# Ogeon/pyrite

Measured on AMD Instinct MI355X. Metric: Msamples/sec, higher is better.
Workload: dtype f32; 1 GPU; C3: c3_mesh_in_box, 1920x1080, 1024 spp; bounces=8, light_samples=4, spectrum_samples=10, spectrum_bins=64, tile_size=32, triangles=819212, spheres=0, parallelism=one launch on one GPU, film_weight_check=ok

## Files before the change

pyrite_amd/csrc/api.cpp:

```cpp
#include <hip/hip_runtime.h>

#include <algorithm>
#include <chrono>
#include <cmath>
#include <cstdlib>
#include <cstring>
#include <memory>
#include <new>
#include <string>
#include <vector>

#include "api_internal.h"
#include "bvh.h"
#include "bvh_device.h"
#include "device_scene.h"
#include "program_regs.h"
#include "scene_internal.h"

using namespace pyr;

namespace pyr {

thread_local std::string g_error;
int fail(int code, const std::string& message) {
// ... 710 lines not shown
            } else if (pr.fast != FAST_NONE) {
                bool seen = false;
                for (size_t j = 0; j < i && !seen; ++j) {
                    const DevProgram& q = programs[j];
                    seen = q.kind == PYR_PROGRAM_INSTRUCTIONS && q.fast == pr.fast && q.fast_spectrum == pr.fast_spectrum && std::memcmp(&q.fast_scale, &pr.fast_scale, sizeof(float)) == 0;
                }
                fast_programs += seen ? 0u : 1u;
            }
        }
    }
    if (needs_interpreter) {
        bool ok = programs.size() <= 128;
        auto colour = [&](uint32_t id) {
            if (id >= programs.size()) return;
            const DevProgram& pr = programs[id];
            if (pr.kind != PYR_PROGRAM_INSTRUCTIONS) return;
            if (pr.tape_form == TAPE_FORM_NONE) ok = false;
            if (pr.tape_form == TAPE_FORM_HIT_RGB) v.rgb_records = 1u;
            if (pr.tape_form == TAPE_FORM_HIT_RGB || pr.tape_form == TAPE_FORM_PRODUCT) v.micro_records = 1u;
            if (pr.tape_form == TAPE_FORM_PRODUCT) v.product_records = 1u;
        };
        for (uint32_t i = 0; i < d->num_components; ++i) colour(d->components[i].color_program);
        for (uint32_t i = 0; i < d->num_lamps; ++i)
            if (d->lamps[i].kind != PYR_LAMP_SHAPE) colour(d->lamps[i].color_program);
        colour(d->sky_program);
        if (tape_rows_needed(fast_programs, v.rgb_records != 0) > kTapeMaxValueRows) ok = false;
        const char* off = std::getenv("PYRITE_HIT_TAPE");
        if (off && off[0] == '0') ok = false;
        if (wide_vm) ok = false;
        v.hit_tape = ok ? 1u : 0u;
        if (!ok) v.rgb_records = v.micro_records = v.product_records = 0u;
    }
    v.tape_value_rows = tape_rows_needed(fast_programs, v.rgb_records != 0) <= kTapeMaxValueRows ? tape_rows_needed(fast_programs, v.rgb_records != 0) : kTapeValueRows;
    v.shadow_margin = d->num_spheres != 0 ? 1.01f : 1.001f;
    v.hero_only_records = 0;
    for (uint32_t i = 0; i < d->num_materials; ++i)
        for (uint32_t k = 0; k < d->materials[i].num_emissive; ++k) {
            const int probability = d->components[d->materials[i].first_emissive + k].probability_program;
            if (probability >= 0 && programs[(size_t)probability].reads_wavelength) v.hero_only_records = 1u;
        }
    v.sphere_tex_scale = (const float*)s->sphere_tex_scale.ptr;
    v.plane_frames = (const float*)s->plane_frames.ptr;
    v.textures = (const DevTexture*)s->textures.ptr;
    v.texture_data = (const float*)s->texture_data.ptr;

    if ((rc = pack_geometry(d, s, builder)) != PYR_OK) return rc;
    s->live.keep(d);
    PyrBuildInfo& build_info = s->build_info;
    build_info.total_ms = (float)ms_between(t_start, std::chrono::steady_clock::now());
    build_info.pack_upload_ms = build_info.total_ms - build_info.bounds_ms - build_info.tree_ms - build_info.finish_ms - build_info.collapse_ms;
    return PYR_OK;
}

uint64_t film_buffer_grains(const PyrFilmDesc* film, const PyrRenderParams* p, const TilePlan& plan) {
    if (p->film_layout == PYR_FILM_TILE_BLOCKS) return (uint64_t)plan.tile_count * (p->tile_size + 2ull) * (p->tile_size + 2ull) * film->bins;
    const uint32_t rows = p->film_row_count ? p->film_row_count : film->height;
    return (uint64_t)rows * film->width * film->bins;
}


int reserve_tape(PyrScene* scene, RenderLaunch& L, hipStream_t stream) {
    const size_t bytes = (size_t)L.tape_lanes * L.tape_max_ops * sizeof(unsigned long long);
    if (bytes > scene->tape.bytes) {
        HIP_TRY(hipStreamSynchronize(stream));
        scene->tape.release();
        int rc = scene->tape.alloc(bytes);
// ... 566 lines not shown
```

pyrite_amd/csrc/device_scene.h:

```cpp
#pragma once
#include <cstddef>
#include <cstdint>

#include "../../include/pyrite_gpu.h"

namespace pyr {

struct DevPrim {
    float a[4], b[4], c[4];
};

struct DevPrimPair {
    float q[5][4];
};

struct DevTriShade {
    float n1[4], n2[4], n3[4];
};

struct DevTriTex {
    float uv12[4], uv3[4], f1[4], f2[4], f3[4];
};

struct DevTexture {
// ... 61 lines not shown
    float rgb_min, rgb_max;
    uint32_t sky_program;
    uint32_t stack_depth;
    uint32_t needs_interpreter;
    uint32_t num_nodes, num_prims;
    uint32_t num_spectra, num_spectrum_floats;
    uint32_t num_programs;
    uint32_t num_materials, num_components;
    uint32_t lds_table_floats;
    const float* tri_tex;
    const float* sphere_tex_scale;
    const float* plane_frames;
    const DevTexture* textures;
    const float* texture_data;
    uint32_t uses_textures;
    uint32_t hero_only_records;
    uint32_t hit_tape;
    uint32_t rgb_records;
    uint32_t product_records;
    uint32_t micro_records;
    float shadow_margin;
    uint32_t tape_value_rows;
};

constexpr uint32_t kTapeValueRows = 8, kTapeOneRow = kTapeValueRows - 1, kTapeMaxValueRows = 16;
constexpr uint32_t tape_row(uint32_t slot) { return slot + (slot >= kTapeOneRow ? 1u : 0u); }
constexpr uint32_t tape_rgb_row(uint32_t n_spectral) { return n_spectral + 3u <= kTapeOneRow ? n_spectral : (n_spectral >= kTapeOneRow ? n_spectral + 1u : kTapeValueRows); }
constexpr uint32_t tape_rows_needed(uint32_t n_spectral, bool rgb) {
    return (rgb ? tape_rgb_row(n_spectral) + 3u : (n_spectral == 0u ? 0u : tape_row(n_spectral - 1u) + 1u)) > kTapeValueRows
               ? (rgb ? tape_rgb_row(n_spectral) + 3u : tape_row(n_spectral - 1u) + 1u)
               : kTapeValueRows;
}

constexpr uint32_t kMaxStackDepth = 64;

struct RenderLaunch {
    PyrCamera camera;
    PyrFilmDesc film;
    uint32_t bounces, light_samples, spectrum_samples, tile_size, pixel_samples;
    uint32_t tiles_x, tiles_y;
    uint32_t tile_begin, tile_stride, tile_count;
    uint32_t chunks_per_tile;
    uint32_t chunk_begin, chunk_end;
    uint32_t film_layout;
    uint32_t film_row_begin, film_row_count;
    uint64_t seed;
    float grains_per_wavelength;
    PyrGrain* film_out;
    unsigned long long* counters;
    uint32_t scheduler;
    uint32_t sm_phase_lanes, sm_trav_steps;
    uint32_t sm_expose_lanes;
    uint32_t stack_lds;
    unsigned long long* tape;
    uint32_t tape_lanes, tape_max_ops;
    uint32_t* tape_overflow;
    uint32_t tape_programs_lds;
    uint32_t sample_begin;
    uint32_t* start_queue;
    uint32_t start_queue_stride;
};

#ifndef PYR_SAMPLE_QUEUE
#define PYR_SAMPLE_QUEUE 1
#endif
constexpr uint32_t kStartQueueEntries = 128, kStartQueueFixedWords = 11;
// ... 207 lines not shown
```

pyrite_amd/csrc/kernels.hip:

```cpp
#ifndef PYRITE_KERNELS_HIP
#define PYRITE_KERNELS_HIP
#include <hip/hip_runtime.h>

#include <algorithm>
#include <cstdint>
#include <cstdlib>
#include <string>
#include <type_traits>

#include "device_scene.h"
#include "exact_math.h"

#ifdef PYR_WIDE_VM
#define PYR_VM_NUMBERS PYR_WIDE_NUMBER_REGISTERS
#define PYR_VM_VECTORS PYR_WIDE_VECTOR_REGISTERS
#define PYR_VM_RGBS PYR_WIDE_RGB_REGISTERS
#else
#define PYR_VM_NUMBERS PYR_MAX_NUMBER_REGISTERS
#define PYR_VM_VECTORS PYR_MAX_VECTOR_REGISTERS
#define PYR_VM_RGBS PYR_MAX_RGB_REGISTERS
#endif
static_assert((PYR_VM_NUMBERS & (PYR_VM_NUMBERS - 1)) == 0 && (PYR_VM_VECTORS & (PYR_VM_VECTORS - 1)) == 0 && (PYR_VM_RGBS & (PYR_VM_RGBS - 1)) == 0,
              "the interpreter masks register indices: its files are powers of two");

// ... 1930 lines not shown
        const uint32_t first = code >> 3, count = code & 7u;
        const ScenePtr<true> pr{view.pairs + 5 * (size_t)first};
        const bool blocks = leaf_pair_test<COUNT>(pr[0], pr[1], pr[2], pr[3], pr[4], count, t, cnt);
        const bool more = count > 2u;
        done = blocks | (!more & (t.sp == 0));
        t.node = more ? -1 - (int)(((first + 1u) << 3) | (count - 2u)) : top;
        t.sp = more ? t.sp : below;
    }
    return done;
}

#ifndef PYR_PRIO_E
#define PYR_PRIO_E 0
#endif
#ifndef PYR_PRIO_S
#define PYR_PRIO_S 1
#endif
#ifndef PYR_PRIO_N
#define PYR_PRIO_N 2
#endif
#ifndef PYR_PRIO_T
#define PYR_PRIO_T 3
#endif
#define PYR_PRIO_ANY (PYR_PRIO_E != PYR_PRIO_S || PYR_PRIO_S != PYR_PRIO_N || PYR_PRIO_N != PYR_PRIO_T)
#if PYR_PRIO_ANY
#define PHASE_PRIO(x) __builtin_amdgcn_s_setprio(x)
#else
#define PHASE_PRIO(x)
#endif

constexpr uint32_t kTapeEagerSlots = 8;
constexpr uint32_t TAPE_MUL = 0u, TAPE_ADD = 1u, TAPE_SCALE = 2u, TAPE_HERO_ONLY = 1u << 29, TAPE_PROGRAM_MASK = (1u << 28) - 1u;
constexpr uint32_t TAPE_EAGER_ADD = 1u << 31, TAPE_EAGER_SLOT_SHIFT = 8, TAPE_EAGER_SLOT_MASK = 0xFu << TAPE_EAGER_SLOT_SHIFT;
constexpr uint32_t kTapeOneSlot = kTapeEagerSlots - 1;
static_assert(kTapeEagerSlots == kTapeValueRows && kTapeOneSlot == kTapeOneRow, "device_scene.h tape_row() and friends");
constexpr uint32_t TAPE_RGB_SHIFT = 12, TAPE_RGB_FIRST = 1u << TAPE_RGB_SHIFT, TAPE_RGB_NEXT = 2u << TAPE_RGB_SHIFT, TAPE_RGB_APPLY = 3u << TAPE_RGB_SHIFT,
                   TAPE_RGB_TIMES = 4u << TAPE_RGB_SHIFT;
static_assert(BLOCK == 1u << TAPE_EAGER_SLOT_SHIFT, "an eager record's slot field is an index into rows of BLOCK floats");

DEV size_t tape_index(uint32_t op, uint32_t lanes, uint32_t column) { return (size_t)op * lanes + column; }
template <bool COUNT, bool INTERP, bool TAPE = false, bool PRODUCT = false>
struct Walker {
    uint32_t stage = ST_NEW;
    uint32_t n_ops = 0;
    uint32_t tape_column = 0;
    const uint32_t* tape_prepared = nullptr;
    DEV void tape_push(const RenderLaunch& L, uint32_t kind, uint32_t program, float s, bool hero_only = false) {
        if (n_ops < L.tape_max_ops) {
            uint32_t word = (kind << 30) | (hero_only ? TAPE_HERO_ONLY : 0u) | (program & TAPE_PROGRAM_MASK);
            if (tape_prepared != nullptr) {
                uint32_t slot = kTapeOneSlot;
                if (kind != TAPE_SCALE) {
                    const uint32_t* e = tape_prepared + 8 * program;
                    if (e[0] == 0u)
                        s = __uint_as_float(e[1]) * s;
                    else
                        slot = e[7];
                }
                word = (kind == TAPE_ADD ? TAPE_EAGER_ADD : 0u) | (hero_only ? TAPE_HERO_ONLY : 0u) | (slot << TAPE_EAGER_SLOT_SHIFT);
            }
            L.tape[tape_index(n_ops, L.tape_lanes, tape_column)] = (unsigned long long)word | ((unsigned long long)__float_as_uint(s) << 32);
        } else {
            *L.tape_overflow = 1u;
        }
        n_ops++;
    }
    DEV void tape_push_raw(const RenderLaunch& L, uint32_t word, float s) {
        if (n_ops < L.tape_max_ops)
            L.tape[tape_index(n_ops, L.tape_lanes, tape_column)] = (unsigned long long)word | ((unsigned long long)__float_as_uint(s) << 32);
        else
            *L.tape_overflow = 1u;
        n_ops++;
    }
    uint32_t rgb_slot = 0;
    static constexpr bool QUEUE = PYR_SAMPLE_QUEUE != 0 && TAPE && !INTERP;
    uint32_t chunk = 0;
    uint32_t q_state = 0;
#ifdef PYR_PHASE_PROFILE
    unsigned long long prof_start[4] = {0, 0, 0, 0};
#endif
    Path p{};
    Trav t{};
    f3 b_position = mk(0, 0, 0), b_normal = mk(0, 0, 0), b_out = mk(0, 0, 0);
    bool b_flip = false;
// ... 372 lines not shown
    for (uint32_t k = 0; k < p.num_instrs; ++k) {
        const PyrInstr& ins = S.instrs[p.first_instr + k];
        float r = 0.0f;
        switch (ins.op) {
        case PYR_OP_NUMBER: r = __uint_as_float(ins.x.bits); break;
        case PYR_OP_SPECTRUM: r = spectrum_get(S, ins.a, value(ins.x)); break;
        case PYR_OP_BLACKBODY: {
            const float wl = value(ins.x), temp = value(ins.y);
            r = blackbody(wl, temp);
            break;
        }
        case PYR_OP_MIX: {
            const float amount = fmaxf(fminf(value(ins.x), 1.0f), 0.0f);
            const float l = num[ins.a & (PYR_MAX_NUMBER_REGISTERS - 1)], rr = num[ins.b & (PYR_MAX_NUMBER_REGISTERS - 1)];
            r = l * (1.0f - amount) + rr * amount;
            break;
        }
        case PYR_OP_BINARY: {
            const float l = num[ins.a & (PYR_MAX_NUMBER_REGISTERS - 1)], rr = num[ins.b & (PYR_MAX_NUMBER_REGISTERS - 1)];
            r = ins.operator_ == PYR_BIN_ADD ? l + rr : (ins.operator_ == PYR_BIN_SUB ? l - rr : (ins.operator_ == PYR_BIN_MUL ? l * rr : l / rr));
            break;
        }
        default: {
            const float v = value(ins.x), mn = value(ins.y), mx = value(ins.z);
            r = fmaxf(fminf(v, mx), mn);
            break;
        }
        }
        num[ins.output & (PYR_MAX_NUMBER_REGISTERS - 1)] = r;
    }
    return num[p.output_reg & (PYR_MAX_NUMBER_REGISTERS - 1)];
}

template <bool COUNT, bool RGB = false, bool TIMES = false>
DEV void replay_tapes(const DevScene& S, const RenderLaunch& L, bool exposing, uint32_t n_ops, uint32_t tape_column, const Path& p, const float* wl_rows,
                      uint32_t wl_column, uint32_t* wave_list, const uint32_t* prepared_lds, float* spectral_values, uint32_t n_spectral, bool eager, Counters& cnt) {
    const uint32_t lane = threadIdx.x & 63u;
    const unsigned long long mask = ballot64(exposing);
    const uint32_t n = (uint32_t)__popcll(mask);
    if (n == 0) return;
    uint32_t max_ops = exposing ? (n_ops < L.tape_max_ops ? n_ops : L.tape_max_ops) : 0u;
    const uint32_t my_ops = max_ops;
    for (int off = 32; off > 0; off >>= 1) max_ops = max(max_ops, (uint32_t)__shfl_xor((int)max_ops, off));
    const bool keeps = exposing && p.use_additional, lost = exposing && !p.use_additional;
    const bool longest = 3u * my_ops > 2u * max_ops, shortest = 3u * my_ops <= max_ops;
    const unsigned long long below = (1ull << lane) - 1ull;
    const unsigned long long k0 = ballot64(keeps && longest), k1 = ballot64(keeps && !longest && !shortest), k2 = ballot64(keeps && shortest);
    const unsigned long long l0 = ballot64(lost && longest), l1 = ballot64(lost && !longest && !shortest), l2 = ballot64(lost && shortest);
    const uint32_t n_full = (uint32_t)__builtin_popcountll(k0 | k1 | k2);
    if (exposing) {
        const unsigned long long mine = keeps ? (longest ? k0 : (shortest ? k2 : k1)) : (longest ? l0 : (shortest ? l2 : l1));
        uint32_t before = keeps ? 0u : n_full;
        before += (uint32_t)__builtin_popcountll(keeps ? ((longest ? 0ull : k0) | (shortest ? k1 : 0ull)) : ((longest ? 0ull : l0) | (shortest ? l1 : 0ull)));
        wave_list[before + (uint32_t)__builtin_popcountll(mine & below)] = lane;
    }
    __builtin_amdgcn_wave_barrier();
    const uint32_t SS = L.spectrum_samples, full_items = n_full * SS, items = full_items + (n - n_full);
    const unsigned long long past_the_end =
        eager ? ((unsigned long long)(kTapeOneSlot << TAPE_EAGER_SLOT_SHIFT) | ((unsigned long long)__float_as_uint(1.0f) << 32)) : 0ull;
#ifndef PYR_REPLAY_ROWS
#define PYR_REPLAY_ROWS 8
#endif
    constexpr uint32_t ROWS = PYR_REPLAY_ROWS;
    for (uint32_t base = 0; base < items; base += 64) {
        const uint32_t i = base + lane;
        const bool active = i < items;
        const bool full = i < full_items;
        const uint32_t rank = !active ? 0u : (full ? i / SS : n_full + (i - full_items)), k = !active ? 0u : (full ? i - rank * SS : SS - 1u);
        const uint32_t src = wave_list[rank];
        const uint32_t ops = (uint32_t)__shfl((int)n_ops, (int)src);
        uint32_t pass_ops = active ? (ops < L.tape_max_ops ? ops : L.tape_max_ops) : 0u;
        for (int off = 32; off > 0; off >>= 1) pass_ops = max(pass_ops, (uint32_t)__shfl_xor((int)pass_ops, off));
        const uint32_t pixel = (uint32_t)__shfl((int)p.pixel, (int)src);
        const float hero_wl = __shfl(p.wl, (int)src);
        const bool hero = k == SS - 1;
        const bool run = active;
        const uint32_t src_column = (uint32_t)__shfl((int)wl_column, (int)src);
        const float wl = hero ? hero_wl : wl_rows[k * BLOCK + src_column];
        float refl = 1.0f, bright = 0.0f, value = 0.0f;
        uint32_t value_of = 0xFFFFFFFFu;
        [[maybe_unused]] float rgb_sum = 0.0f;
        if (eager) {
            const uint32_t* slot_program = prepared_lds + 8 * L.tape_programs_lds;
            uint32_t grid_min = 0, grid_max = 0, grid_count = 0;
            uint32_t i0 = 0, i1 = 0;
            float mix = 0.0f;
            bool below = false, above = false;
            for (uint32_t slot = 0; slot < n_spectral; ++slot) {
                const uint32_t* e = prepared_lds + 8 * slot_program[slot];
                const uint32_t mode = e[0], format = e[2], count = e[6];
                const float c = __uint_as_float(e[1]);
                const float* data = S.spectrum_data + e[5];
                float v;
                if (RGB && mode == 0xFFu) {
                    v = lambda_eval(S, S.programs[slot_program[slot]], wl);
                } else if (format == PYR_SPECTRUM_ARRAY && count != 0u) {
                    if (e[3] != grid_min || e[4] != grid_max || count != grid_count) {
                        grid_min = e[3], grid_max = e[4], grid_count = count;
                        const float lo = __uint_as_float(grid_min), hi = __uint_as_float(grid_max);
                        below = wl <= lo, above = wl >= hi;
                        const float normalized = (wl - lo) / (hi - lo);
                        const float float_index = normalized * ((float)count - 1.0f);
                        const float min_float_index = truncf(float_index);
                        i0 = (below | above) ? 0u : (uint32_t)min_float_index;
                        i1 = (below | above) ? 0u : i0 + 1u;
                        mix = float_index - min_float_index;
                    }
                    const float inside = data[i0] * (1.0f - mix) + data[i1] * mix;
                    v = below ? data[0] : (above ? data[count - 1] : inside);
                } else {
                    PyrSpectrum sp;
                    sp.format = format, sp.min = __uint_as_float(e[3]), sp.max = __uint_as_float(e[4]), sp.offset = e[5], sp.count = count;
                    v = spectrum_eval(sp, data, wl);
                }
                spectral_values[tape_row(slot) * BLOCK] = (mode == FAST_SPECTRUM || mode == 0xFFu) ? v : v * c;
            }
            if (RGB && S.rgb_records != 0) {
                float resp[3] = {0.0f, 0.0f, 0.0f};
                const uint32_t count = S.rgb_count;
                if (count > 0) {
                    const float* d = S.rgb_basis;
                    if (wl <= S.rgb_min) {
                        for (int j = 0; j < 3; ++j) resp[j] = d[j];
                    } else if (wl >= S.rgb_max) {
                        for (int j = 0; j < 3; ++j) resp[j] = d[3 * (count - 1) + j];
                    } else {
                        const float normalized = (wl - S.rgb_min) / (S.rgb_max - S.rgb_min);
                        const float fi = normalized * ((float)count - 1.0f);
                        const float fmin_ = truncf(fi);
                        const uint32_t b0 = (uint32_t)fmin_;
                        const float bmix = fi - fmin_;
                        for (int j = 0; j < 3; ++j) resp[j] = d[3 * b0 + j] * (1.0f - bmix) + d[3 * (b0 + 1) + j] * bmix;
                    }
                }
                for (uint32_t j = 0; j < 3; ++j) spectral_values[(tape_rgb_row(n_spectral) + j) * BLOCK] = resp[j];
            }
        }
        for (uint32_t r0 = 0; r0 < pass_ops; r0 += ROWS) {
            unsigned long long rows[ROWS];
#pragma unroll
            for (uint32_t j = 0; j < ROWS; ++j) rows[j] = r0 + j < my_ops ? L.tape[tape_index(r0 + j, L.tape_lanes, tape_column)] : past_the_end;
            uint32_t words[ROWS];
            float factors[ROWS];
#pragma unroll
            for (uint32_t j = 0; j < ROWS; ++j) {
                words[j] = (uint32_t)__shfl((int)(uint32_t)rows[j], (int)src);
                factors[j] = __uint_as_float((uint32_t)__shfl((int)(uint32_t)(rows[j] >> 32), (int)src));
            }
// ... 56 lines not shown
                if ((word & TAPE_HERO_ONLY) && !hero) continue;
                const uint32_t program = word & TAPE_PROGRAM_MASK;
                if (program != value_of) {
                    Prepared q_prog;
                    if (program < L.tape_programs_lds) {
                        const uint32_t* e = prepared_lds + 8 * program;
                        q_prog.mode = e[0];
                        q_prog.c = __uint_as_float(e[1]);
                        q_prog.sp.format = e[2];
                        q_prog.sp.min = __uint_as_float(e[3]);
                        q_prog.sp.max = __uint_as_float(e[4]);
                        q_prog.sp.offset = e[5];
                        q_prog.sp.count = e[6];
                        q_prog.data = S.spectrum_data + e[5];
                        q_prog.id = program;
                    } else {
                        q_prog = prepare_program<false>(S, program);
                    }
                    VmInput in{wl, mk(0, 0, 0), mk(0, 0, 0)};
                    value = eval_prepared<false>(S, q_prog, in);
                    value_of = program;
                }
                if (kind == TAPE_MUL)
                    refl *= value * s;
                else
                    bright += value * s * refl;
            }
        }
        if (run) expose_grain<COUNT>(L, pixel, wl, bright, cnt);
    }
    __builtin_amdgcn_wave_barrier();
}

DEV uint32_t prepare_tape_tables(const DevScene& S0, const DevScene& S, const RenderLaunch& L, uint32_t* prepared_lds, bool& eager) {
    auto reads_spectrum = [&](uint32_t i) {
        return S0.programs[i].kind != PYR_PROGRAM_CONSTANT && (S0.programs[i].fast != FAST_NONE || (S0.hit_tape != 0 && S0.programs[i].tape_form == TAPE_FORM_LAMBDA));
    };
    auto alike = [&](uint32_t i, uint32_t j) {
        const DevProgram &a = S0.programs[i], &b = S0.programs[j];
        return a.fast != FAST_NONE && a.fast == b.fast && __float_as_uint(a.fast_scale) == __float_as_uint(b.fast_scale) && a.fast_spectrum == b.fast_spectrum;
    };
    auto first_alike = [&](uint32_t i) {
        for (uint32_t j = 0; j < i; ++j)
            if (reads_spectrum(j) && alike(i, j)) return j;
        return i;
    };
    auto slot_of = [&](uint32_t representative) {
        uint32_t slot = 0;
        for (uint32_t j = 0; j < representative; ++j) slot += (reads_spectrum(j) && first_alike(j) == j) ? 1u : 0u;
        return slot;
    };
    uint32_t n_spectral = 0;
    for (uint32_t i = 0; i < L.tape_programs_lds; ++i) n_spectral += (reads_spectrum(i) && first_alike(i) == i) ? 1u : 0u;
    for (uint32_t i = threadIdx.x; i < L.tape_programs_lds; i += BLOCK) {
        const Prepared q = prepare_program<false>(S, i);
        const bool spectral = reads_spectrum(i);
        const uint32_t representative = spectral ? first_alike(i) : i;
        const uint32_t slot = spectral ? slot_of(representative) : 0u;
        uint32_t* e = prepared_lds + 8 * i;
        e[0] = q.mode, e[1] = __float_as_uint(q.c), e[2] = q.sp.format, e[3] = __float_as_uint(q.sp.min), e[4] = __float_as_uint(q.sp.max);
        e[5] = q.sp.offset, e[6] = q.sp.count, e[7] = tape_row(slot);
        if (spectral && representative == i && slot < kTapeMaxValueRows - 1u) prepared_lds[8 * L.tape_programs_lds + slot] = i;
    }
    __syncthreads();
    eager = L.tape_programs_lds != 0 && tape_rows_needed(n_spectral, S0.rgb_records != 0) <= S0.tape_value_rows && (n_spectral != 0 || S0.hit_tape != 0);
    return eager ? n_spectral : 0u;
}

#ifndef PYR_SM_WAVES_INTERP
#define PYR_SM_WAVES_INTERP 3
#endif
constexpr int sm_waves(bool interp) { return interp ? PYR_SM_WAVES_INTERP : PYR_SM_WAVES; }
template <bool COUNT, bool INTERP, bool LDS_SCENE, bool LDS_TABLES, bool HIT_TAPE = false, bool PRODUCT = false>
__global__ __launch_bounds__(BLOCK, sm_waves(INTERP)) void render_kernel_sm(DevScene S0, RenderLaunch L) {
    extern __shared__ float lds[];
    static_assert(INTERP || !HIT_TAPE, "HIT_TAPE is a form of the interpreter build");
    static_assert(HIT_TAPE || !PRODUCT, "PRODUCT is a form of the hit tape (device_scene.h TapeForm)");
    constexpr bool TAPE = !INTERP || HIT_TAPE;
    const uint32_t SS = L.spectrum_samples;
    Spectral spec{lds + threadIdx.x, SS};
    const uint32_t spectral_rows = TAPE ? SS + 1 + S0.tape_value_rows : 3 * SS;
    TravStack stack;
    int deep_levels[LDS_SCENE ? 1 : kMaxStackDepth];
    stack.deep = deep_levels;
    stack.lds = (lds_int*)(reinterpret_cast<int*>(lds + spectral_rows * BLOCK) + threadIdx.x);
    constexpr bool QUEUE = Walker<COUNT, INTERP, TAPE, PRODUCT>::QUEUE;
    stack.lds_entries = QUEUE ? (int)own_scalar(L.stack_lds) : (int)L.stack_lds;
    Counters cnt{};
    const uint32_t lds_base_floats = (spectral_rows + L.stack_lds) * BLOCK;
    const SceneView view = stage_scene<LDS_SCENE>(S0, lds, lds_base_floats, true);
    const DevScene S = stage_tables<LDS_TABLES ? 1 : 0>(S0, lds, lds_base_floats + (LDS_SCENE ? (S0.num_nodes * 16 + S0.num_prims * 12) : 0));

    const uint32_t lane = threadIdx.x & 63u;
    const uint32_t waves_per_block = BLOCK / 64;
    const uint32_t total_waves = gridDim.x * waves_per_block;
    const int phase_lanes = QUEUE ? (int)own_scalar(L.sm_phase_lanes) : (int)L.sm_phase_lanes, trav_steps = QUEUE ? (int)own_scalar(L.sm_trav_steps) : (int)L.sm_trav_steps;
    const int expose_lanes = TAPE ? (QUEUE ? (int)own_scalar(L.sm_expose_lanes) : (int)L.sm_expose_lanes) : phase_lanes;
    Walker<COUNT, INTERP, TAPE, PRODUCT> w;
    w.chunk = L.chunk_begin + blockIdx.x * waves_per_block + (threadIdx.x >> 6);
    w.tape_prepared = nullptr;
    uint32_t* wave_list = reinterpret_cast<uint32_t*>(lds + SS * BLOCK) + (threadIdx.x & ~63u);
    uint32_t* prepared_lds = reinterpret_cast<uint32_t*>(lds + lds_base_floats + (LDS_SCENE ? (S0.num_nodes * 16 + S0.num_prims * 12) : 0) + (LDS_TABLES ? S0.lds_table_floats : 0));
    uint32_t n_spectral = 0;
    bool eager = false;
    float* spectral_values = lds + (SS + 1) * BLOCK + threadIdx.x;
    if constexpr (TAPE) {
        spectral_values[kTapeOneSlot * BLOCK] = 1.0f;
        n_spectral = prepare_tape_tables(S0, S, L, prepared_lds, eager);
        if (eager) w.tape_prepared = prepared_lds;
        w.rgb_slot = tape_rgb_row(n_spectral);
        w.tape_column = blockIdx.x * BLOCK + threadIdx.x;
        if (HIT_TAPE && !eager) *L.tape_overflow = 1u;
    }

    auto scene_view = [&](const RenderLaunch& Lp) {
        if (LDS_SCENE || INTERP) return S;
        const uint32_t rows = (TAPE ? Lp.spectrum_samples + 1 + S0.tape_value_rows : 3 * Lp.spectrum_samples) + Lp.stack_lds;
        return stage_tables<LDS_TABLES ? 1 : 0, false>(scene_from_kernarg(S0), lds, rows * BLOCK);
    };
    PROF_DECL;
    for (;;) {
        int nT = __popcll(ballot64(w.stage == ST_TRAV));
        int nS = __popcll(ballot64(w.stage == ST_SHADE));
        int nN = __popcll(ballot64(w.stage == ST_NEE));
        int nE = __popcll(ballot64(w.stage == ST_EXPOSE || w.stage == ST_NEW));
        if (max(max(nT, nS), max(nN, nE)) == 0) break;

        if (nE >= expose_lanes || nE == max(max(nT, nS), max(nN, nE))) {
            PHASE_PRIO(PYR_PRIO_E);
            PROF_BEGIN(0, w.stage == ST_EXPOSE || w.stage == ST_NEW);
            const RenderLaunch& Lp = launch_from_kernarg(L);
            const DevScene Sp = scene_view(Lp);
            if constexpr (TAPE) {
                [[maybe_unused]] const unsigned long long t_r0 = PROF_NOW();
                replay_tapes<COUNT, HIT_TAPE, PRODUCT>(Sp, Lp, w.stage == ST_EXPOSE, w.n_ops, w.tape_column, w.p, lds, threadIdx.x, wave_list, prepared_lds, spectral_values, n_spectral,
                                              HIT_TAPE ? eager : n_spectral != 0, cnt);
                PROF_ADD(w.prof_start[3], PROF_NOW() - t_r0);
            }
            w.expose_and_restart(Sp, Lp, spec, cnt, lane, total_waves);
            PROF_END(0);
            nT = __popcll(ballot64(w.stage == ST_TRAV));
            nS = __popcll(ballot64(w.stage == ST_SHADE));
            nE = 0;
        }
        if (nS >= phase_lanes || nS == max(max(nT, nS), max(nN, nE))) {
            PHASE_PRIO(PYR_PRIO_S);
            PROF_BEGIN(1, w.stage == ST_SHADE);
            const RenderLaunch& Lp = launch_from_kernarg(L);
            w.shade(scene_view(Lp), Lp, spec, cnt);
            PROF_END(1);
// ... 164 lines not shown
```

pyrite_amd/csrc/kernels/main.hip:

```cpp
#include "../kernels.hip"

#include "../api_internal.h"

namespace pyr {

__global__ __launch_bounds__(BLOCK) void develop_kernel(DevelopLaunch D) {
    const size_t pixels = (size_t)D.film.width * D.film.height;
    const uint32_t bins = D.film.bins;
    const float min = D.film.wl_start, max = D.film.wl_start + D.film.wl_width;
    for (size_t px = (size_t)blockIdx.x * BLOCK + threadIdx.x; px < pixels; px += (size_t)gridDim.x * BLOCK) {
        uint8_t out[3] = {0, 0, 0};
        if ((px + 1) * bins < pixels * bins) {
            const PyrGrain* g = D.grains + px * bins;
            auto xyz_get = [&](int channel, float w) {
                const float* d = D.xyz_table;
                const uint32_t n = D.xyz_count;
                if (w <= D.xyz_min) return d[channel];
                if (w >= D.xyz_max) return d[3 * (n - 1) + channel];
                float normalized = (w - D.xyz_min) / (D.xyz_max - D.xyz_min);
                float fi = normalized * ((float)n - 1.0f);
                float fmin_ = truncf(fi);
                uint32_t i0 = (uint32_t)fmin_;
                float mix = fi - fmin_;
                return d[3 * i0 + channel] * (1.0f - mix) + d[3 * (i0 + 1) + channel] * mix;
// ... 121 lines not shown
}

constexpr size_t kLdsSceneBytes = 8 * 1024;
static bool scene_fits_lds(const DevScene& scene) { return (size_t)scene.num_nodes * 64 + (size_t)scene.num_prims * 48 <= kLdsSceneBytes; }
constexpr uint32_t kShortStackMax = 16;
static uint32_t short_stack_levels(const DevScene& scene, size_t other_bytes, uint32_t workgroups) {
    const char* e = std::getenv("PYRITE_LDS_STACK");
    uint32_t levels;
    if (e && *e) {
        levels = (uint32_t)std::strtoul(e, nullptr, 10);
    } else {
        const size_t budget = (160 * 1024) / std::max(workgroups, 1u);
        levels = budget > other_bytes ? (uint32_t)((budget - other_bytes) / (BLOCK * sizeof(int))) : 0u;
        levels = std::min(levels, kShortStackMax);
    }
    return std::max(1u, std::min(levels, scene.wide_nodes ? scene.wide_stack_depth : scene.stack_depth));
}
uint32_t tape_ops_bound(const DevScene& scene, const RenderLaunch& launch) {
    return (launch.bounces + 2u * launch.light_samples + 1u) * (scene.micro_records ? 4u : 1u) + launch.bounces;
}
uint32_t tape_lanes_bound(int num_cus) { return (uint32_t)num_cus * 8u * BLOCK; }
constexpr uint32_t kTapeProgramsLds = 128;
static uint32_t tape_programs_in_lds(const DevScene& scene) { return scene.num_programs <= kTapeProgramsLds ? scene.num_programs : 0u; }
static bool uses_hit_tape(const DevScene& scene, const RenderLaunch& launch) {
    static const char* const least = std::getenv("PYRITE_HIT_TAPE_WAVELENGTHS");
    return scene.needs_interpreter != 0 && scene.hit_tape != 0 && launch.spectrum_samples >= (least && *least ? (uint32_t)std::strtoul(least, nullptr, 10) : 4u);
}
uint32_t launch_tape(const DevScene& scene, const RenderLaunch& launch) {
    if (launch.scheduler != 1) return 0u;
    return scene.needs_interpreter == 0 ? 1u : uses_hit_tape(scene, launch) ? 2u : 0u;
}
static bool uses_tape(const DevScene& scene, const RenderLaunch& launch) { return launch_tape(scene, launch) != 0u; }
static size_t render_lds_bytes(const DevScene& scene, const RenderLaunch& launch) {
    const size_t spectral_rows = uses_tape(scene, launch) ? launch.spectrum_samples + 1 + scene.tape_value_rows : 3 * launch.spectrum_samples;
    size_t bytes = (spectral_rows + launch.stack_lds) * BLOCK * sizeof(float);
    if (scene_fits_lds(scene)) bytes += (size_t)scene.num_nodes * 64 + (size_t)scene.num_prims * 48;
    bytes += (size_t)scene.lds_table_floats * sizeof(float);
    if (uses_tape(scene, launch)) bytes += ((size_t)tape_programs_in_lds(scene) * 8 + kTapeMaxValueRows) * sizeof(uint32_t);
    return bytes;
}


static RenderKernel pick_kernel(bool sm, bool with_counters, bool interp, bool lds_scene, bool lds_tables, bool hit_tape, bool product, bool wide_vm) {
    if (interp && wide_vm) return pick_wide_kernel(with_counters, lds_scene, lds_tables);
    if (interp) return pick_interp_kernel(with_counters, lds_scene, lds_tables, hit_tape, product);
    auto pick = [&](auto counters) -> RenderKernel {
        constexpr bool C = decltype(counters)::value;
        if (lds_scene) return sm ? render_kernel_sm<C, false, true, false> : render_kernel<C, true, false>;
        if (sm) return lds_tables ? render_kernel_sm<C, false, false, true> : render_kernel_sm<C, false, false, false>;
        return lds_tables ? render_kernel<C, false, true> : render_kernel<C, false, false>;
    };
    return with_counters ? pick(std::true_type{}) : pick(std::false_type{});
}

bool scene_is_lds_resident(const DevScene& scene) { return scene_fits_lds(scene); }

int launch_render(const DevScene& scene, const RenderLaunch& launch_in, bool with_counters, void* stream, int num_cus, bool wide_vm) {
    if (scene.stack_depth > kMaxStackDepth) return fail(PYR_ERR_UNSUPPORTED, "BVH deeper than kMaxStackDepth");
    if (wide_vm && (launch_in.scheduler != 1 || scene.needs_interpreter == 0 || uses_tape(scene, launch_in)))
        return fail(PYR_ERR_INVALID_ARGUMENT, "the wide interpreter build runs the stage scheduler's online form only");
    RenderLaunch launch = launch_in;
    launch.stack_lds = 0;
    launch.tape_programs_lds = uses_tape(scene, launch) ? tape_programs_in_lds(scene) : 0u;
    launch.stack_lds = launch.scheduler == 1 ? short_stack_levels(scene, render_lds_bytes(scene, launch), (uint32_t)sm_waves(scene.needs_interpreter != 0))
                                             : scene.stack_depth;
    if (scene_fits_lds(scene)) launch.stack_lds = std::max(launch.stack_lds, scene.stack_depth);
    const size_t lds = render_lds_bytes(scene, launch);
    if (lds > 160 * 1024) return fail(PYR_ERR_UNSUPPORTED, "spectrum_samples + BVH depth need more than 160 KB of LDS per workgroup");
    const uint32_t chunks = launch.chunk_end - launch.chunk_begin;
    if (chunks == 0) return PYR_OK;
    RenderKernel kernel = pick_kernel(launch.scheduler == 1, with_counters, scene.needs_interpreter != 0, scene_fits_lds(scene), scene.lds_table_floats != 0,
// ... 52 lines not shown
```

Measured before the change: 650.5 Msamples/s.

## Replay hit tapes two wavelengths per lane with paired value rows

For non-interpreter scenes, the tape replay now processes two spectral samples per lane. Spectral values sit in interleaved pair rows, so one tape read and one shuffle feed both wavelengths, halving the number of replay items and tape loads per path. The wave lane list shrinks to bytes and moves after the prepared tables, and the LDS row layout is reshaped to reclaim rows. The cost is more LDS value rows and more branching and register use in the replay loop.

```diff
diff --git a/pyrite_amd/csrc/api.cpp b/pyrite_amd/csrc/api.cpp
--- a/pyrite_amd/csrc/api.cpp
+++ b/pyrite_amd/csrc/api.cpp
@@ -766,6 +766,7 @@
         if (!ok) v.rgb_records = v.micro_records = v.product_records = 0u;
     }
     v.tape_value_rows = tape_rows_needed(fast_programs, v.rgb_records != 0) <= kTapeMaxValueRows ? tape_rows_needed(fast_programs, v.rgb_records != 0) : kTapeValueRows;
+    if (tape_pairs(needs_interpreter)) v.tape_value_rows = tape_pair_build_rows(fast_programs);
     v.shadow_margin = d->num_spheres != 0 ? 1.01f : 1.001f;
     v.hero_only_records = 0;
     for (uint32_t i = 0; i < d->num_materials; ++i)
diff --git a/pyrite_amd/csrc/device_scene.h b/pyrite_amd/csrc/device_scene.h
--- a/pyrite_amd/csrc/device_scene.h
+++ b/pyrite_amd/csrc/device_scene.h
@@ -117,6 +117,24 @@
                : kTapeValueRows;
 }
 
+#ifndef PYR_REPLAY_PAIRS
+#define PYR_REPLAY_PAIRS 1
+#endif
+constexpr bool tape_pairs(bool interpreter) { return PYR_REPLAY_PAIRS != 0 && !interpreter; }
+constexpr uint32_t kTapeOnePair = 1, kTapeMaxPairRows = 2u * kTapeMaxValueRows, kTapePackedOneRow = 2u * kTapeOnePair;
+constexpr uint32_t tape_pair(uint32_t slot) { return slot + (slot >= kTapeOnePair ? 1u : 0u); }
+constexpr uint32_t tape_pair_rows(uint32_t n_spectral) { return 2u * (n_spectral + 1u); }
+constexpr uint32_t tape_packed_row(uint32_t slot) { return slot + (slot >= kTapePackedOneRow ? 1u : 0u); }
+constexpr uint32_t tape_packed_rows(uint32_t n_spectral) { return n_spectral < kTapePackedOneRow ? kTapePackedOneRow + 1u : n_spectral + 1u; }
+constexpr bool tape_pairs_pay(uint32_t n_spectral) { return 2u * n_spectral <= tape_rows_needed(n_spectral, false); }
+constexpr bool tape_replays_pairs(uint32_t n_spectral, uint32_t value_rows) { return tape_pairs_pay(n_spectral) && tape_pair_rows(n_spectral) <= value_rows; }
+constexpr uint32_t tape_pair_build_rows(uint32_t n_spectral) {
+    return tape_pairs_pay(n_spectral) ? tape_pair_rows(n_spectral) : (tape_packed_rows(n_spectral) <= kTapeMaxValueRows ? tape_packed_rows(n_spectral) : 1u);
+}
+constexpr uint32_t tape_first_value_row(uint32_t spectrum_samples, bool interpreter) { return tape_pairs(interpreter) ? spectrum_samples - 1u : spectrum_samples + 1u; }
+constexpr uint32_t tape_spectral_rows(uint32_t spectrum_samples, uint32_t value_rows, bool interpreter) { return tape_first_value_row(spectrum_samples, interpreter) + value_rows; }
+constexpr uint32_t tape_lane_list_bytes(bool interpreter) { return tape_pairs(interpreter) ? 256u : 0u; }
+
 constexpr uint32_t kMaxStackDepth = 64;
 
 struct RenderLaunch {
diff --git a/pyrite_amd/csrc/kernels.hip b/pyrite_amd/csrc/kernels.hip
--- a/pyrite_amd/csrc/kernels.hip
+++ b/pyrite_amd/csrc/kernels.hip
@@ -1986,6 +1986,8 @@
 constexpr uint32_t kTapeEagerSlots = 8;
 constexpr uint32_t TAPE_MUL = 0u, TAPE_ADD = 1u, TAPE_SCALE = 2u, TAPE_HERO_ONLY = 1u << 29, TAPE_PROGRAM_MASK = (1u << 28) - 1u;
 constexpr uint32_t TAPE_EAGER_ADD = 1u << 31, TAPE_EAGER_SLOT_SHIFT = 8, TAPE_EAGER_SLOT_MASK = 0xFu << TAPE_EAGER_SLOT_SHIFT;
+constexpr uint32_t TAPE_PAIR_SLOT_MASK = 0x1Fu << TAPE_EAGER_SLOT_SHIFT;
+static_assert(2u * (kTapeMaxValueRows - 1u) <= 0x1Fu, "a pair record's row field");
 constexpr uint32_t kTapeOneSlot = kTapeEagerSlots - 1;
 static_assert(kTapeEagerSlots == kTapeValueRows && kTapeOneSlot == kTapeOneRow, "device_scene.h tape_row() and friends");
 constexpr uint32_t TAPE_RGB_SHIFT = 12, TAPE_RGB_FIRST = 1u << TAPE_RGB_SHIFT, TAPE_RGB_NEXT = 2u << TAPE_RGB_SHIFT, TAPE_RGB_APPLY = 3u << TAPE_RGB_SHIFT,
@@ -2003,7 +2005,7 @@
         if (n_ops < L.tape_max_ops) {
             uint32_t word = (kind << 30) | (hero_only ? TAPE_HERO_ONLY : 0u) | (program & TAPE_PROGRAM_MASK);
             if (tape_prepared != nullptr) {
-                uint32_t slot = kTapeOneSlot;
+                uint32_t slot = tape_pairs(INTERP) ? kTapePackedOneRow : kTapeOneSlot;
                 if (kind != TAPE_SCALE) {
                     const uint32_t* e = tape_prepared + 8 * program;
                     if (e[0] == 0u)
@@ -2442,9 +2444,9 @@
     return num[p.output_reg & (PYR_MAX_NUMBER_REGISTERS - 1)];
 }
 
-template <bool COUNT, bool RGB = false, bool TIMES = false>
+template <bool COUNT, bool RGB = false, bool TIMES = false, typename LaneNumber = uint32_t>
 DEV void replay_tapes(const DevScene& S, const RenderLaunch& L, bool exposing, uint32_t n_ops, uint32_t tape_column, const Path& p, const float* wl_rows,
-                      uint32_t wl_column, uint32_t* wave_list, const uint32_t* prepared_lds, float* spectral_values, uint32_t n_spectral, bool eager, Counters& cnt) {
+                      uint32_t wl_column, LaneNumber* wave_list, const uint32_t* prepared_lds, float* spectral_values, uint32_t n_spectral, bool eager, Counters& cnt) {
     const uint32_t lane = threadIdx.x & 63u;
     const unsigned long long mask = ballot64(exposing);
     const uint32_t n = (uint32_t)__popcll(mask);
@@ -2462,20 +2464,134 @@
         const unsigned long long mine = keeps ? (longest ? k0 : (shortest ? k2 : k1)) : (longest ? l0 : (shortest ? l2 : l1));
         uint32_t before = keeps ? 0u : n_full;
         before += (uint32_t)__builtin_popcountll(keeps ? ((longest ? 0ull : k0) | (shortest ? k1 : 0ull)) : ((longest ? 0ull : l0) | (shortest ? l1 : 0ull)));
-        wave_list[before + (uint32_t)__builtin_popcountll(mine & below)] = lane;
+        wave_list[before + (uint32_t)__builtin_popcountll(mine & below)] = (LaneNumber)lane;
     }
     __builtin_amdgcn_wave_barrier();
-    const uint32_t SS = L.spectrum_samples, full_items = n_full * SS, items = full_items + (n - n_full);
+    constexpr bool PAIRS = tape_pairs(RGB);
+    const bool paired = PAIRS && eager && tape_replays_pairs(n_spectral, S.tape_value_rows);
+    const uint32_t SS = L.spectrum_samples, per_path = paired ? (SS + 1u) / 2u : SS, full_items = n_full * per_path, items = full_items + (n - n_full);
     const unsigned long long past_the_end =
-        eager ? ((unsigned long long)(kTapeOneSlot << TAPE_EAGER_SLOT_SHIFT) | ((unsigned long long)__float_as_uint(1.0f) << 32)) : 0ull;
-#ifndef PYR_REPLAY_ROWS
-#define PYR_REPLAY_ROWS 8
+        eager ? ((unsigned long long)((PAIRS ? kTapePackedOneRow : kTapeOneSlot) << TAPE_EAGER_SLOT_SHIFT) | ((unsigned long long)__float_as_uint(1.0f) << 32)) : 0ull;
+#ifndef PYR_REPLAY_PAIR_ROWS
+#define PYR_REPLAY_PAIR_ROWS 4
 #endif
-    constexpr uint32_t ROWS = PYR_REPLAY_ROWS;
+#ifdef PYR_REPLAY_ROWS
+    constexpr uint32_t ROWS = PYR_REPLAY_ROWS, PAIR_ROWS = PYR_REPLAY_PAIR_ROWS;
+#else
+    constexpr uint32_t ROWS = PAIRS ? 4 : 8, PAIR_ROWS = PYR_REPLAY_PAIR_ROWS;
+#endif
     for (uint32_t base = 0; base < items; base += 64) {
         const uint32_t i = base + lane;
         const bool active = i < items;
         const bool full = i < full_items;
+        if (paired) {
+            const uint32_t rank = !active ? 0u : (full ? i / per_path : n_full + (i - full_items)), ka = !active ? 0u : (full ? i - rank * per_path : SS - 1u), kb = ka + per_path;
+            const uint32_t src = wave_list[rank];
+            const uint32_t ops = (uint32_t)__shfl((int)n_ops, (int)src);
+            uint32_t pass_ops = active ? (ops < L.tape_max_ops ? ops : L.tape_max_ops) : 0u;
+            for (int off = 32; off > 0; off >>= 1) pass_ops = max(pass_ops, (uint32_t)__shfl_xor((int)pass_ops, off));
+            const uint32_t pixel = (uint32_t)__shfl((int)p.pixel, (int)src);
+            const float hero_wl = __shfl(p.wl, (int)src);
+            const bool hero_a = ka == SS - 1, hero_b = kb == SS - 1;
+            const uint32_t pixel_a = active ? pixel : PIXEL_NONE, pixel_b = active && kb < SS ? pixel : PIXEL_NONE;
+            const uint32_t not_for_a = hero_a ? 0u : TAPE_HERO_ONLY, not_for_b = hero_b ? 0u : TAPE_HERO_ONLY;
+            const uint32_t src_column = (uint32_t)__shfl((int)wl_column, (int)src);
+            const float wl_a = hero_a ? hero_wl : wl_rows[ka * BLOCK + src_column];
+            const float wl_b = hero_b ? hero_wl : (kb < SS ? wl_rows[(kb < SS ? kb : ka) * BLOCK + src_column] : wl_a);
+            const f2v wl = {wl_a, wl_b};
+            f2v refl = {1.0f, 1.0f}, bright = {0.0f, 0.0f};
+            {
+                const uint32_t* slot_program = prepared_lds + 8 * L.tape_programs_lds;
+                uint32_t grid_min = 0, grid_max = 0, grid_count = 0;
+                uint32_t i0[2] = {0, 0}, i1[2] = {0, 0};
+                float mix[2] = {0.0f, 0.0f};
+                uint32_t edge[2] = {0, 0};
+                for (uint32_t slot = 0; slot < n_spectral; ++slot) {
+                    const uint32_t* e = prepared_lds + 8 * slot_program[slot];
+                    const uint32_t mode = e[0], format = e[2], count = e[6];
+                    const float c = __uint_as_float(e[1]);
+                    const float* data = S.spectrum_data + e[5];
+                    float v[2] = {0.0f, 0.0f};
+                    if (format == PYR_SPECTRUM_ARRAY && count != 0u) {
+                        if (e[3] != grid_min || e[4] != grid_max || count != grid_count) {
+                            grid_min = e[3], grid_max = e[4], grid_count = count;
+                            const float lo = __uint_as_float(grid_min), hi = __uint_as_float(grid_max);
+#pragma unroll
+                            for (uint32_t h = 0; h < 2; ++h) {
+                                const bool under = wl[h] <= lo, above = wl[h] >= hi;
+                                edge[h] = under ? 1u : (above ? 2u : 0u);
+                                const float normalized = (wl[h] - lo) / (hi - lo);
+                                const float float_index = normalized * ((float)count - 1.0f);
+                                const float min_float_index = truncf(float_index);
+                                i0[h] = (under | above) ? 0u : (uint32_t)min_float_index;
+                                i1[h] = (under | above) ? 0u : i0[h] + 1u;
+                                mix[h] = float_index - min_float_index;
+                            }
+                        }
+#pragma unroll
+                        for (uint32_t h = 0; h < 2; ++h) {
+                            const float inside = data[i0[h]] * (1.0f - mix[h]) + data[i1[h]] * mix[h];
+                            v[h] = edge[h] == 1u ? data[0] : (edge[h] == 2u ? data[count - 1] : inside);
+                        }
+                    } else {
+                        PyrSpectrum sp;
+                        sp.format = format, sp.min = __uint_as_float(e[3]), sp.max = __uint_as_float(e[4]), sp.offset = e[5], sp.count = count;
+#pragma nounroll
+                        for (uint32_t h = 0; h < 2; ++h) {
+                            const float one = spectrum_eval(sp, data, h == 0u ? wl_a : wl_b);
+                            v[0] = h == 0u ? one : v[0], v[1] = one;
+                        }
+                    }
+#pragma unroll
+                    for (uint32_t h = 0; h < 2; ++h) spectral_values[(2u * tape_pair(slot) + h) * BLOCK] = mode == FAST_SPECTRUM ? v[h] : v[h] * c;
+                }
+            }
+            for (uint32_t r0 = 0; r0 < pass_ops; r0 += PAIR_ROWS) {
+                unsigned long long rows[PAIR_ROWS];
+#pragma unroll
+                for (uint32_t j = 0; j < PAIR_ROWS; ++j) rows[j] = r0 + j < my_ops ? L.tape[tape_index(r0 + j, L.tape_lanes, tape_column)] : past_the_end;
+                uint32_t words[PAIR_ROWS];
+                float factors[PAIR_ROWS];
+#pragma unroll
+                for (uint32_t j = 0; j < PAIR_ROWS; ++j) {
+                    words[j] = (uint32_t)__shfl((int)(uint32_t)rows[j], (int)src);
+                    factors[j] = __uint_as_float((uint32_t)__shfl((int)(uint32_t)(rows[j] >> 32), (int)src));
+                }
+                f2v values[PAIR_ROWS];
+#pragma unroll
+                for (uint32_t j = 0; j < PAIR_ROWS; ++j) {
+                    const float* row = spectral_values + (words[j] & TAPE_PAIR_SLOT_MASK);
+                    values[j] = f2v{row[0], row[BLOCK]};
+                }
+                if (S.hero_only_records == 0) {
+#pragma unroll
+                    for (uint32_t j = 0; j < PAIR_ROWS; ++j) {
+                        const f2v m = values[j] * factors[j];
+                        const bool adds = (int)words[j] < 0;
+                        const f2v multiplied = refl * m, added = bright + multiplied;
+                        bright.x = adds ? added.x : bright.x, bright.y = adds ? added.y : bright.y;
+                        refl.x = adds ? refl.x : multiplied.x, refl.y = adds ? refl.y : multiplied.y;
+                    }
+                    continue;
+                }
+#pragma unroll
+                for (uint32_t j = 0; j < PAIR_ROWS; ++j) {
+                    const f2v product = values[j] * factors[j];
+                    const uint32_t skip_a = 0u - ((words[j] & not_for_a) >> 29), skip_b = 0u - ((words[j] & not_for_b) >> 29);
+                    static_assert(TAPE_HERO_ONLY == 1u << 29, "the shift above");
+                    const f2v m = {__uint_as_float((__float_as_uint(product.x) & ~skip_a) | (__float_as_uint(1.0f) & skip_a)),
+                                   __uint_as_float((__float_as_uint(product.y) & ~skip_b) | (__float_as_uint(1.0f) & skip_b))};
+                    const bool adds_a = (int)(words[j] & ~skip_a) < 0, adds_b = (int)(words[j] & ~skip_b) < 0;
+                    const f2v multiplied = refl * m, added = bright + multiplied;
+                    bright.x = adds_a ? added.x : bright.x, bright.y = adds_b ? added.y : bright.y;
+                    refl.x = adds_a ? refl.x : multiplied.x, refl.y = adds_b ? refl.y : multiplied.y;
+                }
+            }
+#pragma nounroll
+            for (uint32_t h = 0; h < 2; ++h)
+                expose_grain<COUNT>(L, h == 0u ? pixel_a : pixel_b, h == 0u ? wl_a : wl_b, h == 0u ? bright.x : bright.y, cnt);
+            continue;
+        }
         const uint32_t rank = !active ? 0u : (full ? i / SS : n_full + (i - full_items)), k = !active ? 0u : (full ? i - rank * SS : SS - 1u);
         const uint32_t src = wave_list[rank];
         const uint32_t ops = (uint32_t)__shfl((int)n_ops, (int)src);
@@ -2523,7 +2639,7 @@
                     sp.format = format, sp.min = __uint_as_float(e[3]), sp.max = __uint_as_float(e[4]), sp.offset = e[5], sp.count = count;
                     v = spectrum_eval(sp, data, wl);
                 }
-                spectral_values[tape_row(slot) * BLOCK] = (mode == FAST_SPECTRUM || mode == 0xFFu) ? v : v * c;
+                spectral_values[(PAIRS ? tape_packed_row(slot) : tape_row(slot)) * BLOCK] = (mode == FAST_SPECTRUM || mode == 0xFFu) ? v : v * c;
             }
             if (RGB && S.rgb_records != 0) {
                 float resp[3] = {0.0f, 0.0f, 0.0f};
@@ -2646,6 +2762,7 @@
     __builtin_amdgcn_wave_barrier();
 }
 
+template <bool PAIRS>
 DEV uint32_t prepare_tape_tables(const DevScene& S0, const DevScene& S, const RenderLaunch& L, uint32_t* prepared_lds, bool& eager) {
     auto reads_spectrum = [&](uint32_t i) {
         return S0.programs[i].kind != PYR_PROGRAM_CONSTANT && (S0.programs[i].fast != FAST_NONE || (S0.hit_tape != 0 && S0.programs[i].tape_form == TAPE_FORM_LAMBDA));
@@ -2666,6 +2783,7 @@
     };
     uint32_t n_spectral = 0;
     for (uint32_t i = 0; i < L.tape_programs_lds; ++i) n_spectral += (reads_spectrum(i) && first_alike(i) == i) ? 1u : 0u;
+    const bool paired = PAIRS && tape_replays_pairs(n_spectral, S0.tape_value_rows);
     for (uint32_t i = threadIdx.x; i < L.tape_programs_lds; i += BLOCK) {
         const Prepared q = prepare_program<false>(S, i);
         const bool spectral = reads_spectrum(i);
@@ -2673,11 +2791,12 @@
         const uint32_t slot = spectral ? slot_of(representative) : 0u;
         uint32_t* e = prepared_lds + 8 * i;
         e[0] = q.mode, e[1] = __float_as_uint(q.c), e[2] = q.sp.format, e[3] = __float_as_uint(q.sp.min), e[4] = __float_as_uint(q.sp.max);
-        e[5] = q.sp.offset, e[6] = q.sp.count, e[7] = tape_row(slot);
+        e[5] = q.sp.offset, e[6] = q.sp.count, e[7] = !PAIRS ? tape_row(slot) : (paired ? 2u * tape_pair(slot) : tape_packed_row(slot));
         if (spectral && representative == i && slot < kTapeMaxValueRows - 1u) prepared_lds[8 * L.tape_programs_lds + slot] = i;
     }
     __syncthreads();
-    eager = L.tape_programs_lds != 0 && tape_rows_needed(n_spectral, S0.rgb_records != 0) <= S0.tape_value_rows && (n_spectral != 0 || S0.hit_tape != 0);
+    eager = L.tape_programs_lds != 0 && (paired || (PAIRS ? tape_packed_rows(n_spectral) : tape_rows_needed(n_spectral, S0.rgb_records != 0)) <= S0.tape_value_rows) &&
+            (n_spectral != 0 || S0.hit_tape != 0);
     return eager ? n_spectral : 0u;
 }
 
@@ -2693,7 +2812,7 @@
     constexpr bool TAPE = !INTERP || HIT_TAPE;
     const uint32_t SS = L.spectrum_samples;
     Spectral spec{lds + threadIdx.x, SS};
-    const uint32_t spectral_rows = TAPE ? SS + 1 + S0.tape_value_rows : 3 * SS;
+    const uint32_t spectral_rows = TAPE ? tape_spectral_rows(SS, S0.tape_value_rows, INTERP) : 3 * SS;
     TravStack stack;
     int deep_levels[LDS_SCENE ? 1 : kMaxStackDepth];
     stack.deep = deep_levels;
@@ -2713,14 +2832,20 @@
     Walker<COUNT, INTERP, TAPE, PRODUCT> w;
     w.chunk = L.chunk_begin + blockIdx.x * waves_per_block + (threadIdx.x >> 6);
     w.tape_prepared = nullptr;
-    uint32_t* wave_list = reinterpret_cast<uint32_t*>(lds + SS * BLOCK) + (threadIdx.x & ~63u);
     uint32_t* prepared_lds = reinterpret_cast<uint32_t*>(lds + lds_base_floats + (LDS_SCENE ? (S0.num_nodes * 16 + S0.num_prims * 12) : 0) + (LDS_TABLES ? S0.lds_table_floats : 0));
+    typedef std::conditional_t<tape_pairs(INTERP), uint8_t, uint32_t> LaneNumber;
+    LaneNumber* wave_list = (tape_pairs(INTERP) ? reinterpret_cast<LaneNumber*>(prepared_lds + 8 * L.tape_programs_lds + kTapeMaxValueRows) : reinterpret_cast<LaneNumber*>(lds + SS * BLOCK)) +
+                            (threadIdx.x & ~63u);
     uint32_t n_spectral = 0;
     bool eager = false;
-    float* spectral_values = lds + (SS + 1) * BLOCK + threadIdx.x;
+    float* spectral_values = lds + tape_first_value_row(SS, INTERP) * BLOCK + threadIdx.x;
     if constexpr (TAPE) {
-        spectral_values[kTapeOneSlot * BLOCK] = 1.0f;
-        n_spectral = prepare_tape_tables(S0, S, L, prepared_lds, eager);
+        if constexpr (!tape_pairs(INTERP)) spectral_values[kTapeOneSlot * BLOCK] = 1.0f;
+        n_spectral = prepare_tape_tables<tape_pairs(INTERP)>(S0, S, L, prepared_lds, eager);
+        if (tape_pairs(INTERP) && eager) {
+            spectral_values[kTapePackedOneRow * BLOCK] = 1.0f;
+            if (tape_replays_pairs(n_spectral, S0.tape_value_rows)) spectral_values[(kTapePackedOneRow + 1u) * BLOCK] = 1.0f;
+        }
         if (eager) w.tape_prepared = prepared_lds;
         w.rgb_slot = tape_rgb_row(n_spectral);
         w.tape_column = blockIdx.x * BLOCK + threadIdx.x;
@@ -2729,7 +2854,7 @@
 
     auto scene_view = [&](const RenderLaunch& Lp) {
         if (LDS_SCENE || INTERP) return S;
-        const uint32_t rows = (TAPE ? Lp.spectrum_samples + 1 + S0.tape_value_rows : 3 * Lp.spectrum_samples) + Lp.stack_lds;
+        const uint32_t rows = (TAPE ? tape_spectral_rows(Lp.spectrum_samples, S0.tape_value_rows, INTERP) : 3 * Lp.spectrum_samples) + Lp.stack_lds;
         return stage_tables<LDS_TABLES ? 1 : 0, false>(scene_from_kernarg(S0), lds, rows * BLOCK);
     };
     PROF_DECL;
diff --git a/pyrite_amd/csrc/kernels/main.hip b/pyrite_amd/csrc/kernels/main.hip
--- a/pyrite_amd/csrc/kernels/main.hip
+++ b/pyrite_amd/csrc/kernels/main.hip
@@ -177,11 +177,11 @@
 }
 static bool uses_tape(const DevScene& scene, const RenderLaunch& launch) { return launch_tape(scene, launch) != 0u; }
 static size_t render_lds_bytes(const DevScene& scene, const RenderLaunch& launch) {
-    const size_t spectral_rows = uses_tape(scene, launch) ? launch.spectrum_samples + 1 + scene.tape_value_rows : 3 * launch.spectrum_samples;
+    const size_t spectral_rows = uses_tape(scene, launch) ? tape_spectral_rows(launch.spectrum_samples, scene.tape_value_rows, scene.needs_interpreter != 0) : 3 * launch.spectrum_samples;
     size_t bytes = (spectral_rows + launch.stack_lds) * BLOCK * sizeof(float);
     if (scene_fits_lds(scene)) bytes += (size_t)scene.num_nodes * 64 + (size_t)scene.num_prims * 48;
     bytes += (size_t)scene.lds_table_floats * sizeof(float);
-    if (uses_tape(scene, launch)) bytes += ((size_t)tape_programs_in_lds(scene) * 8 + kTapeMaxValueRows) * sizeof(uint32_t);
+    if (uses_tape(scene, launch)) bytes += ((size_t)tape_programs_in_lds(scene) * 8 + kTapeMaxValueRows) * sizeof(uint32_t) + tape_lane_list_bytes(scene.needs_interpreter != 0);
     return bytes;
 }
 
```

After: 665.5 Msamples/s (median of 6 runs). +2.3%, better.
